# gwenzhang/GGA

Hardware: AMD Instinct MI355X
Metric: kitti_frames_per_sec_gga_train_step (higher is better)
Workload: dtype f32 tensors; products on 2 x f16 operand planes (block-scaled), f32 accumulate - measured no less accurate than fp32 kernels: per convolution 0.7 x (dense) / 0.7-1.2 x (sparse) the RMS error of an fp32 FMA chain vs float64, whole-step losses over 8 seeds <= 2.5e-5 from float64 (fp32 CPU step: <= 1.6

## Files before the change

gga_amd/_lib.py:

```python
import ctypes as C
import os
import subprocess

_HERE = os.path.dirname(os.path.abspath(__file__))
LIB_PATH = os.path.join(_HERE, 'libgga_hip.so')
ABI_VERSION = 36

_lib = None

vp, i32, i64, f32, sz = C.c_void_p, C.c_int, C.c_int64, C.c_float, C.c_size_t
I3 = C.POINTER(C.c_int32 * 3)


class VoxelParams(C.Structure):
    _fields_ = [('voxel_size', C.c_float * 3), ('pc_range', C.c_float * 6),
                ('max_points', C.c_int32), ('max_voxels', C.c_int32)]


class PfnParams(C.Structure):
    _fields_ = [('voxel_size', C.c_float * 3), ('offsets', C.c_float * 3), ('eps', C.c_float),
                ('momentum', C.c_float), ('training', C.c_int32), ('in_features', C.c_int32),
                ('channels', C.c_int32)]


# ... 52 lines not shown
CENTER_MAX_K = 512


class CenterParams(C.Structure):
    _fields_ = [('pc_range', C.c_float * 2), ('voxel_size', C.c_float * 2), ('out_size_factor', C.c_float),
                ('gaussian_overlap', C.c_float), ('min_radius', C.c_int32), ('K', C.c_int32), ('H', C.c_int32), ('W', C.c_int32),
                ('n_tasks', C.c_int32), ('n_classes', C.c_int32), ('task_classes', C.c_int32 * MAX_TASKS),
                ('task_class_base', C.c_int32 * MAX_TASKS), ('class_task', C.c_int32 * CENTER_MAX_CLASSES),
                ('class_index', C.c_int32 * CENTER_MAX_CLASSES)]


class CenterLossTask(C.Structure):
    _fields_ = [('pred', vp), ('anno_box', vp), ('mask', vp), ('loss', vp), ('grad_loss', vp), ('grad_pred', vp)]


class CenterLossTable(C.Structure):
    _fields_ = [('n_tasks', C.c_int32), ('task', CenterLossTask * MAX_TASKS)]


class CenterLossWeights(C.Structure):
    _fields_ = [('code_weights', C.c_float * 8), ('loss_weight', C.c_float)]


FPS_REGISTER_MAX_N = 20480
GROUP_MAX_SAMPLES = 256
ANCHOR_MAX_GROUPS = 16
ANCHOR_LOSS_WORKSPACE_BYTES = 24576


class AnchorParams(C.Structure):
    _fields_ = [('n_groups', C.c_int32), ('n_rot', C.c_int32), ('num_classes', C.c_int32), ('assign_per_class', C.c_int32),
                ('pos_iou_thr', C.c_float * ANCHOR_MAX_GROUPS), ('neg_iou_thr', C.c_float * ANCHOR_MAX_GROUPS),
                ('min_pos_iou', C.c_float * ANCHOR_MAX_GROUPS), ('pos_weight', C.c_float), ('dir_offset', C.c_float),
                ('dir_limit_offset', C.c_float)]


class AnchorLossParams(C.Structure):
    _fields_ = [('B', C.c_int32), ('HW', C.c_int32), ('n_anchors', C.c_int32), ('num_classes', C.c_int32),
                ('diff_rad_by_sin', C.c_int32), ('reserved', C.c_int32), ('cls_stride', C.c_int64 * 3),
                ('reg_stride', C.c_int64 * 3), ('dir_stride', C.c_int64 * 3), ('gamma', C.c_float), ('alpha', C.c_float),
                ('beta', C.c_float), ('code_weight', C.c_float * 7), ('loss_weight', C.c_float * 3)]


class LossParams(C.Structure):
    _fields_ = [('B', C.c_int32), ('K', C.c_int32), ('fm_w', C.c_int32),
                ('voxel_size', C.c_float * 2), ('out_size_factor', C.c_float),
                ('pc_range', C.c_float * 2), ('code_weights', C.c_float * 5),
                ('l1_loss_weight', C.c_float), ('w_bpl', C.c_float), ('w_srl', C.c_float),
                ('w_pal', C.c_float)]


SIGNATURES = {
    'gga_last_error': (C.c_char_p, []),
    'gga_abi_version': (i32, []),
    'gga_timing_begin': (i32, [i32, i32, i64]),
    'gga_timing_collect': (i32, [i32, vp, i32]),
    'gga_voxel_grid_size': (None, [C.POINTER(VoxelParams), C.POINTER(C.c_int32 * 3)]),
    'gga_hard_voxelize_workspace_bytes': (sz, [i32, i64]),
    'gga_hard_voxelize_batch': (i32, [vp, i32, C.POINTER(C.c_int64), i32, C.POINTER(VoxelParams),
                                       vp, vp, vp, vp, vp, sz, vp]),
    'gga_hard_voxelize_prepared': (i32, [vp, i32, C.POINTER(C.c_int64), vp, i32, C.POINTER(VoxelParams),
                                          vp, vp, vp, vp, vp, sz, vp]),
    'gga_dynamic_voxelize': (i32, [vp, i32, C.POINTER(C.c_int64), vp, i32, C.POINTER(VoxelParams), vp, vp, vp]),
    'gga_dynamic_voxel_map_workspace_bytes': (sz, [i64]),
    'gga_dynamic_voxel_map': (i32, [vp, vp, i32, i64, i32, i32, i32, i32, vp, vp, vp, vp, vp, vp, sz, vp]),
    'gga_dynamic_scatter_chunk': (i32, []),
    'gga_dynamic_scatter_workspace_bytes': (sz, [i64, i32]),
    'gga_dynamic_scatter_fwd': (i32, [vp, i32, i64, vp, vp, vp, vp, i64, i32, vp, vp, vp, sz, vp]),
    'gga_dynamic_scatter_bwd': (i32, [vp, i32, i64, vp, vp, vp, i64, i32, vp, vp]),
    'gga_dynamic_pfn_workspace_bytes': (sz, [i64]),
    'gga_dynamic_pfn_fwd': (i32, [vp, vp, i64, vp, vp, vp, vp, i64, C.POINTER(PfnParams)] + [vp] * 10 + [sz, vp]),
    'gga_dynamic_pfn_bwd': (i32, [vp, vp, i64, vp, i64, C.POINTER(PfnParams)] + [vp] * 11 + [sz, vp]),
    'gga_points_prepare_workspace_bytes': (sz, [i32, i64, i64]),
    'gga_points_prepare_batch': (i32, [vp, C.POINTER(C.c_int64), vp, C.POINTER(C.c_int64), vp, C.POINTER(C.c_int64),
                                        i32, i32, C.c_double, vp, C.POINTER(C.c_uint64), vp, vp, vp, sz, vp]),
    'gga_voxel_mean': (i32, [vp, vp, i64, i32, i32, i32, vp, vp]),
    'gga_pfn_workspace_bytes': (sz, [i64]),
    'gga_pfn_fwd': (i32, [vp, vp, vp, i64, vp, i32, C.POINTER(PfnParams), vp, vp, vp, vp, vp, vp, vp, vp, vp, sz, vp]),
    'gga_pfn_bwd': (i32, [vp, vp, vp, i64, vp, i32, C.POINTER(PfnParams), vp, vp, vp, vp, vp, vp, vp, vp, vp, vp, sz, vp]),
    'gga_pillar_scatter_map_bytes': (sz, [i32, i32, i32]),
    'gga_pillar_scatter_fwd': (i32, [vp, vp, i64, vp, i32, i32, i32, i32, i32, i32, vp, vp, vp]),
    'gga_pillar_scatter_bwd': (i32, [vp, vp, i64, vp, i32, i32, i32, i32, i32, vp, vp]),
    'gga_pillar_conv_map': (i32, [vp, i64, vp, i32, i32, i32, i32, i32, i32, i32, i32, i32, vp, vp]),
    'gga_sparse_index_bytes': (sz, [i64]),
    'gga_sparse_build_index': (i32, [vp, i64, i32, i32, i32, i32, vp, sz, vp]),
    'gga_sparse_out_index_bytes': (sz, [i64, i32]),
    'gga_sparse_out_sites_workspace_bytes': (sz, [i64, i32]),
    'gga_sparse_conv_out_sites': (i32, [vp, i64, i32, I3, I3, I3, I3, I3, vp, i64, vp, vp, sz, vp, sz, vp]),
    'gga_sparse_rulebook': (i32, [vp, i64, vp, i64, i32, I3, I3, I3, I3, I3, vp, i64, vp, i64, vp, vp, vp]),
    'gga_sparse_rowmask': (i32, [vp, i64, i32, vp, vp]),
    'gga_sparse_mask_order_workspace_bytes': (sz, [i64]),
    'gga_sparse_morton_order_workspace_bytes': (sz, [i64]),
    'gga_sparse_morton_order': (i32, [vp, i64, i32, i32, vp, vp, sz, vp]),
    'gga_sparse_mask_order': (i32, [vp, i64, i32, vp, vp, sz, vp]),
    'gga_sparse_split_weight_bytes': (sz, [i32, i32, i32]),
    'gga_sparse_conv_wgrad_workspace_bytes': (sz, [i64, i32, i32, i32]),
    'gga_dense_wgrad3x3_workspace_bytes': (sz, [i32, i32, i32, i32, i32]),
    'gga_sparse_pack_weight_planes': (i32, [vp, i32, i32, i32, i32, i32, vp, vp, vp]),
    'gga_sparse_conv_apply_tiles': (i64, [i64]),
    'gga_sparse_conv_apply_bn_bwd': (i32, [vp, vp, vp, vp, vp, i64, i32, i32, i32, i32, vp, i64, i32, vp, vp, vp, vp, i64, vp, vp, vp, vp, vp]),
    'gga_sparse_bev_nhwc_fwd': (i32, [vp, vp, i64, i32, i32, i32, i32, i32, vp, vp]),
    'gga_sparse_bev_nhwc_bwd': (i32, [vp, vp, i64, i32, i32, i32, i32, i32, vp, vp]),
    'gga_sparse_halo_tile_rows': (i64, []),
    'gga_sparse_halo_build': (i32, [vp, vp, i64, i64, i32, i32, vp, vp, vp, vp]),
    'gga_sparse_conv_apply_halo': (i32, [vp, vp, vp, vp, i32, vp, vp, i64, i64, i32, i32, i32, i32, vp, i64, i32, vp, vp, vp, vp, i64, vp, vp, vp, vp, vp]),
    'gga_sparse_conv_wgrad_planes': (i32, [vp, i64, vp, i64, vp, i64, i32, i32, i32, vp, i32, vp, vp, vp, sz, vp]),
    'gga_deconv_stream_tiles': (i64, [i64, i32, i32]),
    'gga_deconv_stream_fwd': (i32, [vp, vp, vp, vp, i32, i32, i32, i32, i32, i32, vp, vp, vp]),
    'gga_deconv_stream_bwd': (i32, [vp, vp, vp, vp, i32, i32, i32, i32, i32, i32, vp, vp]),
    'gga_absmax_bits': (i32, [vp, i64, i32, i64, vp, vp]),
    'gga_dense_conv3x3_pack_planes': (i32, [vp, i64, i64, i64, i64, i32, i32, i32, i32, vp, vp, vp]),
    'gga_dense_conv3x3_levels': (i32, [i32, vp, vp, vp, vp, i32, i32, i32, vp, i64, i32, vp, vp, vp, i32, i32, vp, vp]),
    'gga_dense_conv3x3_bn_bwd_pays': (i32, [i32, i32, i32, i32]),
    'gga_dense_conv3x3_bn_bwd_pays_planes': (i32, [i32, i32, i32, i32, i32]),
    'gga_dense_conv3x3_bn_bwd': (i32, [vp, vp, i32, i32, i32, i32, i32, vp, i64, i32, vp, i32, vp, vp, vp, i64, vp, vp, vp, vp, vp]),
    'gga_absmax_table_blocks': (i64, [i64]),
    'gga_absmax_table': (i32, [vp, i32, i64, vp, i32, vp]),
    'gga_pack_weights_table': (i32, [vp, i32, i64, i32, vp]),
    'gga_dense_wgrad3x3_block_amax': (i32, [vp, vp, i32, i32, i32, i32, i32, vp, i64, i64, i64, i64, i32, i32, vp, i32, vp, i32, vp, sz, vp]),
    'gga_dense_conv3x3_tile_rows': (i32, [i32, i32, i32, i32, i32]),
    'gga_dense_conv3x3_stat_rows': (i64, [i32, i32, i32, i32, i32, i32]),
    'gga_bn_relu_workspace_bytes': (sz, [i64, i32]),
    'gga_bn_relu_mask_bytes': (sz, [i64, i32]),
    'gga_bn_relu_fwd': (i32, [vp, vp, vp, vp, vp, vp, i64, i32, f32, f32, i32, i32, vp, i64, vp, vp, vp, i32, vp, vp, sz, vp]),
    'gga_bn_relu_bwd': (i32, [vp, i64, vp, vp, vp, vp, i64, i32, i32, i32, vp, vp, vp, vp, vp, vp, sz, vp]),
    'gga_column_sums': (i32, [vp, i64, i32, vp, vp, sz, vp]),
    'gga_bn_relu_bwd_partials': (i32, [vp, i64, vp, vp, vp, i64, i32, i32, vp, i32, vp, vp, vp, vp, vp, sz, vp]),
    'gga_gn_relu_workspace_bytes': (sz, [i32, i32]),
    'gga_gn_relu_fwd': (i32, [vp, vp, vp, i32, i64, i32, i32, f32, i32, vp, vp, vp, vp, vp, sz, vp]),
    'gga_gn_relu_bwd': (i32, [vp, vp, vp, vp, vp, i32, i64, i32, i32, i32, vp, vp, vp, vp, vp, sz, vp]),
    'gga_bn_stats': (i32, [vp, vp, vp, vp, vp, i64, i32, f32, f32, i32, vp, vp, vp, i32, i32, i32, vp, sz, vp]),
    'gga_head_conv3x3_fwd': (i32, [vp, i64, vp, vp, vp, i32, i32, i32, i32, i32, vp, vp]),
    'gga_head_conv3x3_fwd_tiles': (i32, [vp, i64, vp, vp, vp, i32, i32, i32, i32, i32, vp, vp, vp]),
    'gga_head_cell_tiles_count': (i64, [i32, i32, i32]),
    'gga_head_cell_tiles': (i32, [vp, i32, i32, i32, i32, vp, vp]),
    'gga_head_conv3x3_workspace_bytes': (sz, [i32]),
    'gga_head_conv3x3_wgrad': (i32, [vp, i64, vp, vp, i32, i32, i32, i32, i32, vp, vp, vp, sz, vp]),
    'gga_head_tail_bwd': (i32, [vp, vp, i64, vp, vp, vp, vp, i32, i32, i32, i32, i32, vp, i64, vp, vp, vp, vp, sz, vp]),
    'gga_head_tile_activity': (i32, [vp, i32, i32, i32, i32, vp, vp]),
    'gga_head_branch_bwd_workspace_bytes': (sz, [i32, i32, i32, i32]),
    'gga_head_branch_bwd': (i32, [vp, vp, i64, vp, vp, vp, vp, i32, i32, i32, i32, i32, vp, vp, vp, i64, vp, vp, vp, i32, vp, sz, vp]),
    'gga_heatmap_splat': (i32, [vp, i32, i32, i32, vp, i32, vp, vp, i32, vp]),
    'gga_focal_loss_workspace_bytes': (sz, [i64, i32]),
    'gga_focal_loss_fwd': (i32, [C.POINTER(TaskTable), f32, f32, f32, vp, sz, vp]),
    'gga_focal_loss_bwd': (i32, [C.POINTER(TaskTable), f32, f32, f32, vp]),
    'gga_gather_pred_fwd': (i32, [C.POINTER(TaskTable), i32, i32, i32, i32, vp]),
    'gga_gather_pred_bwd': (i32, [C.POINTER(TaskTable), i32, i32, i32, i32, vp]),
    'gga_box_losses_workspace_bytes': (sz, [i32, i32, i32]),
    'gga_box_losses_fwd': (i32, [C.POINTER(TaskTable), C.POINTER(LossParams), vp, sz, vp]),
    'gga_box_losses_bwd': (i32, [C.POINTER(TaskTable), i32, i32, vp]),
    'gga_center_targets': (i32, [vp, vp, vp, i32, C.POINTER(CenterParams), vp, vp, vp, vp, vp, vp, i32, vp]),
    'gga_center_reg_loss_fwd': (i32, [C.POINTER(CenterLossTable), i32, i32, C.POINTER(CenterLossWeights), vp]),
    'gga_center_reg_loss_bwd': (i32, [C.POINTER(CenterLossTable), i32, i32, C.POINTER(CenterLossWeights), vp]),
    'gga_anchor_targets_workspace_bytes': (sz, [i64, i32]),
    'gga_anchor_targets': (i32, [vp, i32, C.POINTER(AnchorParams), vp, vp, i32, vp, vp, i32, vp, vp, vp, vp, vp, vp, vp, vp, sz, vp]),
    'gga_anchor_loss_fwd': (i32, [C.POINTER(AnchorLossParams), vp, vp, vp, vp, vp, vp, vp, vp, vp, vp, vp, vp, sz, vp]),
    'gga_anchor_loss_bwd': (i32, [C.POINTER(AnchorLossParams), vp, vp, vp, vp, vp, vp, vp, vp, vp, vp, vp, vp, vp, vp, vp]),
    'gga_anchor_decode': (i32, [vp, i32, i32, vp, i32, i32, i32, vp, vp, C.POINTER(C.c_int64 * 3), vp, C.POINTER(C.c_int64 * 3), vp, vp, vp, vp]),
    'gga_box_iou_rotated': (i32, [vp, i32, vp, i32, i32, i32, vp, vp]),
    'gga_nms_rotated_workspace_bytes': (sz, [i32]),
    'gga_nms_rotated_sorted': (i32, [vp, i32, f32, i32, vp, vp, vp, sz, vp]),
    'gga_circle_nms_sorted': (i32, [vp, i32, C.c_double, i32, vp, vp, vp, sz, vp]),
    'gga_region_grow_workspace_bytes': (sz, [i64, i32]),
    'gga_region_grow': (i32, [vp, i64, i32, vp, vp, vp, i32, C.c_double, i32, vp, vp, sz, vp]),
    'gga_points_in_convex_polyhedra': (i32, [vp, i64, i32, vp, vp, i32, i32, vp, vp]),
    'gga_plane_inliers': (i32, [vp, i64, i32, vp, i32, C.c_double, vp, vp, vp]),
# ... 87 lines not shown
```

gga_amd/csrc/scatter.hip:

```cpp
#include "gga_common.h"

__global__ __launch_bounds__(256) void scatter_map_kernel(const int32_t* __restrict__ coors, int64_t m,
                                                         const int32_t* __restrict__ num_valid, int batch,
                                                         int ny, int nx, int32_t* __restrict__ cell_map) {
    const int64_t v = (int64_t)blockIdx.x * 256 + threadIdx.x;
    const int64_t lim = num_valid ? (int64_t)*num_valid : m;
    if (v >= m || v >= lim) return;
    const int4 c = reinterpret_cast<const int4*>(coors)[v];
    if ((unsigned)c.x >= (unsigned)batch || (unsigned)c.z >= (unsigned)ny || (unsigned)c.w >= (unsigned)nx) return;
    atomicMax(&cell_map[((int64_t)c.x * ny + c.z) * nx + c.w], (int32_t)v);
}

template <int UNROLL>
__global__ __launch_bounds__(256) void scatter_canvas_nchw_v1_kernel(const float* __restrict__ feats,
                                                                    int32_t* __restrict__ cell_map, int channels,
                                                                    int64_t cells, int64_t cells4_total,
                                                                    float* __restrict__ canvas) {
    const int64_t q = (int64_t)blockIdx.x * 256 + threadIdx.x;
    if (q >= cells4_total) return;
    const int64_t cells4 = cells >> 2;
    const int64_t b = q / cells4;
    const int64_t cq = q - b * cells4;
    int4* mp = reinterpret_cast<int4*>(cell_map) + q;
    const int4 idx = *mp;
// ... 286 lines not shown
    const int ky = k / kw, kx = k - ky * kw;
    int32_t v = -1;
    if (!num_valid || r < *num_valid) {
        const int4 c = coors[r];
        const int ty = c.z + ph - ky, tx = c.w + pw - kx;
        if (ty >= 0 && tx >= 0 && ty % sh == 0 && tx % sw == 0) {
            const int oy = ty / sh, ox = tx / sw;
            if (oy < oh && ox < ow) v = (c.x * oh + oy) * ow + ox;
        }
    }
    map[(int64_t)k * m + r] = v;
}

__global__ __launch_bounds__(256) void sparse_bev_nhwc_fwd_kernel(const float4* __restrict__ f, const int4* __restrict__ coors,
                                                                int64_t n, int c4n, int D, int H, int W, float* __restrict__ out) {
    const int64_t i = (int64_t)blockIdx.x * 256 + threadIdx.x;
    if (i >= n * c4n) return;
    const int64_t row = i / c4n;
    const int c4 = (int)(i - row * c4n);
    const int4 c = coors[row];
    const float4 v = f[i];
    float* dst = out + (((int64_t)c.x * H + c.z) * W + c.w) * (4 * c4n * D) + (int64_t)(4 * c4) * D + c.y;
    dst[0] = v.x; dst[D] = v.y; dst[2 * D] = v.z; dst[3 * D] = v.w;
}

__global__ __launch_bounds__(256) void sparse_bev_nhwc_bwd_kernel(const float* __restrict__ g, const int4* __restrict__ coors,
                                                                int64_t n, int c4n, int D, int H, int W, float4* __restrict__ gf) {
    const int64_t i = (int64_t)blockIdx.x * 256 + threadIdx.x;
    if (i >= n * c4n) return;
    const int64_t row = i / c4n;
    const int c4 = (int)(i - row * c4n);
    const int4 c = coors[row];
    const float* src = g + (((int64_t)c.x * H + c.z) * W + c.w) * (4 * c4n * D) + (int64_t)(4 * c4) * D + c.y;
    gf[i] = make_float4(src[0], src[D], src[2 * D], src[3 * D]);
}

extern "C" int gga_sparse_bev_nhwc_fwd(const float* feats, const int32_t* coors, int64_t n, int batch, int channels, int depth,
                                       int height, int width, float* out, void* stream_) {
    hipStream_t stream = (hipStream_t)stream_;
    GGA_REQUIRE(out && batch >= 1 && channels >= 4 && channels % 4 == 0 && depth >= 1 && height >= 1 && width >= 1 && n >= 0,
                "gga_sparse_bev_nhwc_fwd: bad sizes (channels %% 4 == 0)");
    GGA_CHECK_HIP(hipMemsetAsync(out, 0, (size_t)batch * height * width * channels * depth * sizeof(float), stream),
                  "gga_sparse_bev_nhwc_fwd: memset");
    if (n == 0) return GGA_OK;
    GGA_REQUIRE(feats && coors && ((uintptr_t)feats & 15) == 0 && ((uintptr_t)coors & 15) == 0, "gga_sparse_bev_nhwc_fwd: null or unaligned pointer");
    const int64_t total = n * (channels / 4);
    hipLaunchKernelGGL(sparse_bev_nhwc_fwd_kernel, dim3((unsigned)((total + 255) / 256)), dim3(256), 0, stream,
                       (const float4*)feats, (const int4*)coors, n, channels / 4, depth, height, width, out);
    GGA_CHECK_LAUNCH("sparse_bev_nhwc_fwd_kernel");
    return GGA_OK;
}

extern "C" int gga_sparse_bev_nhwc_bwd(const float* grad_out, const int32_t* coors, int64_t n, int batch, int channels, int depth,
                                       int height, int width, float* grad_feats, void* stream_) {
    hipStream_t stream = (hipStream_t)stream_;
    GGA_REQUIRE(batch >= 1 && channels >= 4 && channels % 4 == 0 && depth >= 1 && height >= 1 && width >= 1 && n >= 0,
                "gga_sparse_bev_nhwc_bwd: bad sizes (channels %% 4 == 0)");
    if (n == 0) return GGA_OK;
    GGA_REQUIRE(grad_out && coors && grad_feats && ((uintptr_t)grad_feats & 15) == 0 && ((uintptr_t)coors & 15) == 0,
                "gga_sparse_bev_nhwc_bwd: null or unaligned pointer");
    const int64_t total = n * (channels / 4);
    hipLaunchKernelGGL(sparse_bev_nhwc_bwd_kernel, dim3((unsigned)((total + 255) / 256)), dim3(256), 0, stream, grad_out,
                       (const int4*)coors, n, channels / 4, depth, height, width, (float4*)grad_feats);
    GGA_CHECK_LAUNCH("sparse_bev_nhwc_bwd_kernel");
    return GGA_OK;
}

extern "C" int gga_pillar_conv_map(const int32_t* coors, int64_t m, const int32_t* num_valid, int batch, int ny, int nx,
                                   int kh, int kw, int stride_h, int stride_w, int pad_h, int pad_w, int32_t* map,
                                   void* stream) {
    GGA_REQUIRE(coors && map, "gga_pillar_conv_map: null pointer argument");
    GGA_REQUIRE(m >= 0 && batch >= 1 && ny >= 1 && nx >= 1 && kh >= 1 && kw >= 1 && kh * kw <= 65535 && stride_h >= 1 &&
                    stride_w >= 1 && pad_h >= 0 && pad_w >= 0,
                "gga_pillar_conv_map: bad sizes");
    const int oh = (ny + 2 * pad_h - kh) / stride_h + 1, ow = (nx + 2 * pad_w - kw) / stride_w + 1;
    GGA_REQUIRE(oh >= 1 && ow >= 1 && (int64_t)batch * oh * ow < 2147483647ll, "gga_pillar_conv_map: output %dx%d", oh, ow);
    if (m == 0) return GGA_OK;
    hipLaunchKernelGGL(pillar_conv_map_kernel, dim3((unsigned)((m + 255) / 256), kh * kw), dim3(256), 0,
                       (hipStream_t)stream, (const int4*)coors, m, num_valid, kh, kw, stride_h, stride_w, pad_h, pad_w,
                       oh, ow, map);
    GGA_CHECK_LAUNCH("pillar_conv_map_kernel");
    return GGA_OK;
}
```

gga_amd/pillar_conv.py:

```python
import torch
from torch import nn

from . import _lib
from . import functional as F
from . import gather_gemm as G
from ._lib import check


class PillarSupport:
    __slots__ = ('feats', 'coors', 'num_valid')

    def __init__(self, feats, coors, num_valid):
        self.feats, self.coors, self.num_valid = feats, coors, num_valid


def eligible(conv, canvas):
    sup = getattr(canvas, 'pillar_support', None)
    return (sup is not None and type(conv) is nn.Conv2d and conv.bias is None and conv.groups == 1
            and tuple(conv.dilation) == (1, 1) and conv.padding_mode == 'zeros' and not isinstance(conv.padding, str)
            and canvas.is_cuda and canvas.dtype == torch.float32 and torch.is_grad_enabled()
            and (sup.feats.requires_grad or conv.weight.requires_grad)
            and conv.in_channels <= 128 and conv.out_channels <= 128 and conv.in_channels % 4 == 0
            and canvas.is_contiguous(memory_format=torch.channels_last))


class _PillarConv2d(torch.autograd.Function):
    @staticmethod
    def forward(ctx, feats, weight, canvas, coors, num_valid, stride, padding):
        from . import strided_conv
        kh, kw = weight.shape[2:]
        if (strided_conv.ENABLED and kh == kw and stride[0] == stride[1] and padding[0] == padding[1] and stride[0] > 1
                and kh <= 5 and weight.shape[0] % 4 == 0):
            B, Ci, ny, nx = canvas.shape
            bk = strided_conv.book(B, ny, nx, kh, stride[0], padding[0], canvas.device)
            y, stats = G.apply(canvas.permute(0, 2, 3, 1).reshape(-1, Ci), bk.fwd, weight.detach().permute(2, 3, 1, 0).reshape(kh * kw, Ci, -1),
                               bk.n_out, planes=G.planes(), x_amax=G.amax(feats.detach().contiguous()), want_stats=True)
            y = y.view(B, bk.Ho, bk.Wo, -1).permute(0, 3, 1, 2)
        else:
            y = torch.conv2d(canvas, weight, None, stride, padding)
            stats = torch.empty(0, dtype=torch.float64, device=y.device)
        ctx.save_for_backward(feats, weight, coors, num_valid)
        ctx.geom = (tuple(canvas.shape), stride, padding)
        ctx.mark_non_differentiable(stats)
        ctx.set_materialize_grads(False)
        return y, stats

    @staticmethod
    def backward(ctx, gy, _gstats=None):
        feats, w, coors, num_valid = ctx.saved_tensors
        (B, Ci, ny, nx), (sh, sw), (ph, pw) = ctx.geom
        Co, _, kh, kw = w.shape
        kvol, m = kh * kw, feats.shape[0]
        gy = gy.contiguous(memory_format=torch.channels_last)
        rows = gy.permute(0, 2, 3, 1).reshape(-1, Co)
        feats = feats.contiguous()
        L = _lib.lib()
        nbr = torch.empty((kvol, m), dtype=torch.int32, device=gy.device)
        check(L.gga_pillar_conv_map(F._p(coors), m, F._p(num_valid), B, ny, nx, kh, kw, sh, sw, ph, pw, F._p(nbr),
                                    F._stream()), 'gga_pillar_conv_map')
        gx = gw = None
        if ctx.needs_input_grad[0]:
            rb = G.Rulebook(nbr)
            wk = w.permute(2, 3, 0, 1).reshape(kvol, Co, Ci).contiguous()
            gx = G.apply(rows, rb, wk, m, planes=3)
        if ctx.needs_input_grad[1]:
            gw = G.wgrad(rows, feats, nbr, m, planes=3).view(kh, kw, Co, Ci).permute(2, 3, 0, 1)
        return gx, gw, None, None, None, None, None


def pillar_conv2d(canvas, conv):
    sup = canvas.pillar_support
    coors = sup.coors if sup.coors.dtype == torch.int32 else sup.coors.int()
    y, stats = _PillarConv2d.apply(sup.feats, conv.weight, canvas.detach(), coors.contiguous(), sup.num_valid,
                                   tuple(conv.stride), tuple(conv.padding))
    if stats.numel():
        F.attach_bn_partials(y, stats)
    return y
```

gga_amd/strided_conv.py:

```python
import ctypes as C
import os

import torch
from torch import nn

from . import _lib
from . import functional as F
from . import gather_gemm as G
from ._lib import check

ENABLED = True
STREAM = os.environ.get('GGA_DECONV_STREAM', '1') != '0'
STREAM_OFF = set()
_BOOKS = {}


class _Book:

    def __init__(self, B, H, W, k, s, p, device):
        Ho, Wo = (H + 2 * p - k) // s + 1, (W + 2 * p - k) // s + 1
        self.Ho, self.Wo, self.kvol = Ho, Wo, k * k
        self.n_in, self.n_out = B * H * W, B * Ho * Wo
        self._geom = (B, H, W, k, s, p, device)

# ... 106 lines not shown
    from . import dense_conv, weight_bank
    L = _lib.lib()
    B, cout, Hs, Ws = gy.shape
    H, W = Hs // s, Ws // s
    cin = weight.shape[0]
    w_koi = weight.detach().permute(2, 3, 1, 0)
    if dense_conv.RANGE_GUARD.armed:
        dense_conv.RANGE_GUARD.record(w_koi)
    ops = [weight_bank.gather_operand(w_koi, 2, c0, min(c0 + 128, cin)) for c0 in range(0, cin, 128)]
    g_amax = G.amax(gy) if g_amax is None else g_amax
    gx = torch.empty((B, H, W, cin), dtype=torch.float32, device=gy.device)
    check(L.gga_deconv_stream_bwd(F._p(_rows(gy)), _block_pointers([op for op, _ in ops]), F._p(g_amax), F._p(ops[0][1]), B, H, W,
                                  cin, cout, s, F._p(gx), F._stream()), 'gga_deconv_stream_bwd')
    return gx


class _Deconv(torch.autograd.Function):

    @staticmethod
    def forward(ctx, x, weight, s):
        B, cin, H, W = x.shape
        w = weight.detach()
        x_amax = G.amax(x)
        if _stream_form(cin, weight.shape[1], s, False):
            y, stats = _stream_fwd(x, weight, s, x_amax)
            ctx.save_for_backward(x, weight)
            ctx.s, ctx.amax = s, (x_amax, None)
            ctx.mark_non_differentiable(stats)
            ctx.set_materialize_grads(False)
            return y.permute(0, 3, 1, 2), stats
        bk = book(B, H * s, W * s, s, s, 0, x.device)
        y, stats = G.apply(_rows(x), bk.bwd, w.permute(2, 3, 0, 1), bk.n_in, planes=G.planes(), x_amax=x_amax, want_stats=True, bank=True)
        ctx.save_for_backward(x, weight)
        ctx.s, ctx.amax = s, (x_amax, None)
        ctx.mark_non_differentiable(stats)
        ctx.set_materialize_grads(False)
        return y.view(B, H * s, W * s, -1).permute(0, 3, 1, 2), stats

    @staticmethod
    def backward(ctx, gy, _gstats=None):
        x, weight = ctx.saved_tensors
        s = ctx.s
        B, cin, H, W = x.shape
        cout = weight.shape[1]
        gy = gy.contiguous(memory_format=torch.channels_last)
        g_rows = _rows(gy)
        gx = gw = None
        x_amax, w_amax = ctx.amax if G.planes() == 2 else (None, None)
        g_amax = G.amax(gy)
        stream = _stream_form(cin, cout, s, True)
        if not stream or ctx.needs_input_grad[1]:
            bk = book(B, H * s, W * s, s, s, 0, x.device)
        if ctx.needs_input_grad[0]:
            if stream:
                gx = _stream_bwd(gy, weight, s, g_amax).permute(0, 3, 1, 2)
            else:
                w = weight.detach()
                gx = G.apply(g_rows, bk.fwd, w.permute(2, 3, 1, 0), bk.n_out, planes=G.planes(), x_amax=g_amax, bank=True)
                gx = gx.view(B, H, W, cin).permute(0, 3, 1, 2)
        if ctx.needs_input_grad[1]:
            gw = G.wgrad(g_rows, _rows(x), bk.fwd.nbr, bk.n_out, planes=G.planes(), x_amax=g_amax, g_amax=x_amax).view(s, s, cout, cin).permute(3, 2, 0, 1)
        return gx, gw, None


def _common(m, x):
    return (ENABLED and max(m.in_channels, m.out_channels) <= 256 and m.bias is None and m.groups == 1 and m.dilation == (1, 1) and x.is_cuda and x.dtype == torch.float32
            and x.dim() == 4 and x.is_contiguous(memory_format=torch.channels_last) and m.in_channels % 4 == 0
            and m.out_channels % 4 == 0 and x.shape[0] * x.shape[2] * x.shape[3] * max(m.stride) ** 2 < 2 ** 31)


def eligible(m, x):
    if type(m) is nn.Conv2d:
        k, s, p = m.kernel_size, m.stride, m.padding
        return (_common(m, x) and m.padding_mode == 'zeros' and k[0] == k[1] and s[0] == s[1] and p[0] == p[1] and k[0] <= 5
                and (s[0] > 1 or k[0] == 1) and isinstance(p[0], int))
    if type(m) is nn.ConvTranspose2d:
        k, s = m.kernel_size, m.stride
        return (_common(m, x) and k == s and k[0] == k[1] and k[0] <= 5 and m.padding == (0, 0) and m.output_padding == (0, 0))
    return False


def conv(x, m):
    if type(m) is nn.Conv2d:
        y, stats = _StridedConv.apply(x, m.weight, m.kernel_size[0], m.stride[0], m.padding[0])
    else:
        y, stats = _Deconv.apply(x, m.weight, m.stride[0])
    F.attach_bn_partials(y, stats)
    return y
```

include/gga_hip.h:

```cpp
#ifndef GGA_HIP_H_
#define GGA_HIP_H_

#include <stddef.h>
#include <stdint.h>

#ifdef __cplusplus
extern "C" {
#endif

typedef enum {
    GGA_OK = 0,
    GGA_ERR_INVALID_ARG = -1,
    GGA_ERR_WORKSPACE = -2,
    GGA_ERR_LAUNCH = -3
} gga_status;

const char* gga_last_error(void);
int gga_abi_version(void);

enum {
    GGA_TIME_SCATTER_FWD = 0,
    GGA_TIME_DENSE_CONV = 1,
    GGA_TIME_SPARSE_CONV = 2,
    GGA_TIME_SPARSE_WGRAD = 3,
// ... 27 lines not shown
                               void* workspace, size_t workspace_bytes, void* stream);

size_t gga_points_prepare_workspace_bytes(int n_frames, int64_t total_rows, int64_t max_frame_rows);
int gga_points_prepare_batch(const float* scene, const int64_t* scene_offsets_host, const float* sampled,
                             const int64_t* sampled_offsets_host, const double* centers_xy,
                             const int64_t* center_offsets_host, int n_frames, int ndim, double min_distance,
                             const float* pc_range_dev, const uint64_t* shuffle_seeds_host, float* out_points,
                             int32_t* out_counts, void* workspace, size_t workspace_bytes, void* stream);

int gga_voxel_mean(const float* voxels, const int32_t* num_points, int64_t m, int max_points,
                   int ndim, int num_features, float* out, void* stream);

int gga_dynamic_voxelize(const float* points, int ndim, const int64_t* offsets_host, const int32_t* counts_dev, int batch,
                         const gga_voxel_params* prm, int32_t* coors, uint32_t* keys, void* stream);

size_t gga_dynamic_voxel_map_workspace_bytes(int64_t n_points);
int gga_dynamic_voxel_map(const uint32_t* keys, const int32_t* coors, int coor_cols, int64_t n_points, int batch, int grid_x,
                          int grid_y, int grid_z, int32_t* voxel_coors, int32_t* voxel_start, int32_t* order,
                          int32_t* point2voxel, int32_t* counts, void* workspace, size_t workspace_bytes, void* stream);

enum { GGA_DYNAMIC_MEAN = 0, GGA_DYNAMIC_MAX = 1 };
int gga_dynamic_scatter_chunk(void);
size_t gga_dynamic_scatter_workspace_bytes(int64_t n_points, int channels);
int gga_dynamic_scatter_fwd(const float* feats, int channels, int64_t n_points, const int32_t* order,
                            const int32_t* point2voxel, const int32_t* voxel_start, const int32_t* counts, int64_t out_rows,
                            int mode, float* out, int32_t* argmax, void* workspace, size_t workspace_bytes, void* stream);
int gga_dynamic_scatter_bwd(const float* grad_out, int channels, int64_t n_points, const int32_t* point2voxel,
                            const int32_t* voxel_start, const int32_t* argmax, int64_t out_rows, int mode, float* grad_in,
                            void* stream);

typedef struct {
    float voxel_size[3];
    float offsets[3];
    float eps, momentum;
    int32_t training;
    int32_t in_features;
    int32_t channels;
} gga_pfn_params;

size_t gga_pfn_workspace_bytes(int64_t m);
int gga_pfn_fwd(const float* voxels, const int32_t* num_points, const int32_t* coors, int64_t m,
                const int32_t* num_valid, int max_points, const gga_pfn_params* prm, const float* weight, const float* gamma,
                const float* beta, float* running_mean, float* running_var, float* out,
                uint8_t* argmax, double* saved, void* workspace, size_t workspace_bytes,
                void* stream);
int gga_pfn_bwd(const float* voxels, const int32_t* num_points, const int32_t* coors, int64_t m,
                const int32_t* num_valid, int max_points, const gga_pfn_params* prm, const float* weight, const float* gamma,
                const float* out, const uint8_t* argmax, const double* saved, const float* grad_out,
                float* grad_weight, float* grad_gamma, float* grad_beta, void* workspace,
                size_t workspace_bytes, void* stream);

size_t gga_dynamic_pfn_workspace_bytes(int64_t n_points);
int gga_dynamic_pfn_fwd(const float* points, const int32_t* coors, int64_t n_points, const int32_t* order,
                        const int32_t* point2voxel, const int32_t* voxel_start, const int32_t* counts, int64_t out_rows,
                        const gga_pfn_params* prm, const float* weight, const float* gamma, const float* beta,
                        float* running_mean, float* running_var, float* out, int32_t* argmax, float* mean, double* saved,
                        void* workspace, size_t workspace_bytes, void* stream);
int gga_dynamic_pfn_bwd(const float* points, const int32_t* coors, int64_t n_points, const int32_t* counts, int64_t out_rows,
                        const gga_pfn_params* prm, const float* weight, const float* gamma, const float* out,
                        const int32_t* argmax, const float* mean, const double* saved, const float* grad_out,
                        float* grad_weight, float* grad_gamma, float* grad_beta, void* workspace, size_t workspace_bytes,
                        void* stream);

enum { GGA_LAYOUT_NCHW = 0, GGA_LAYOUT_NHWC = 1 };

size_t gga_pillar_scatter_map_bytes(int batch, int ny, int nx);

int gga_pillar_scatter_fwd(const float* feats, const int32_t* coors, int64_t m,
                           const int32_t* num_valid, int batch, int channels, int ny, int nx,
                           int layout, int unique_coors, int32_t* cell_map, float* canvas, void* stream);

int gga_pillar_scatter_bwd(const float* grad_canvas, const int32_t* coors, int64_t m,
                           const int32_t* num_valid, int batch, int channels, int ny, int nx,
                           int layout, float* grad_feats, void* stream);

int gga_sparse_bev_nhwc_fwd(const float* feats, const int32_t* coors, int64_t n, int batch, int channels, int depth, int height,
                            int width, float* out, void* stream);
int gga_sparse_bev_nhwc_bwd(const float* grad_out, const int32_t* coors, int64_t n, int batch, int channels, int depth,
                            int height, int width, float* grad_feats, void* stream);

int gga_pillar_conv_map(const int32_t* coors, int64_t m, const int32_t* num_valid, int batch, int ny, int nx,
                        int kh, int kw, int stride_h, int stride_w, int pad_h, int pad_w, int32_t* map,
                        void* stream);


size_t gga_sparse_index_bytes(int64_t n);
int gga_sparse_build_index(const int32_t* coors, int64_t n, int B, int D, int H, int W, void* index,
                           size_t index_bytes, void* stream);

size_t gga_sparse_out_index_bytes(int64_t n_in, int kvol);
size_t gga_sparse_out_sites_workspace_bytes(int64_t n_in, int kvol);
int gga_sparse_conv_out_sites(const int32_t* in_coors, int64_t n_in, int B, const int32_t in_dhw[3],
                              const int32_t kernel[3], const int32_t stride[3], const int32_t pad[3],
                              int32_t out_dhw[3], int32_t* out_coors, int64_t cap_out, int32_t* n_out,
                              void* out_index, size_t out_index_bytes, void* workspace,
                              size_t workspace_bytes, void* stream);

int gga_sparse_rulebook(const int32_t* out_coors, int64_t n_out, const int32_t* in_coors, int64_t n_in,
                        int B, const int32_t in_dhw[3], const int32_t out_dhw[3], const int32_t kernel[3],
                        const int32_t stride[3], const int32_t pad[3], const void* in_index,
                        int64_t in_index_n, const void* out_index, int64_t out_index_n, int32_t* nbr,
                        int32_t* nbr_t, void* stream);

int gga_sparse_rowmask(const int32_t* map, int64_t n_rows, int kvol, uint32_t* mask, void* stream);
size_t gga_sparse_morton_order_workspace_bytes(int64_t n_rows);
int gga_sparse_morton_order(const int32_t* coors, int64_t n_rows, int batch_size, int max_extent, int32_t* order,
                            void* workspace, size_t workspace_bytes, void* stream);
size_t gga_sparse_mask_order_workspace_bytes(int64_t n_rows);
int gga_sparse_mask_order(const uint32_t* mask, int64_t n_rows, int kvol, int32_t* order, void* workspace,
                          size_t workspace_bytes, void* stream);

size_t gga_sparse_split_weight_bytes(int kvol, int cin, int cout);

int64_t gga_dense_conv3x3_stat_rows(int B, int H, int W, int cout, int planes, int n_slices);
int gga_dense_conv3x3_tile_rows(int B, int H, int W, int cout, int planes);

int gga_absmax_bits(const float* x, int64_t rows, int width, int64_t row_stride, uint32_t* out_bits, void* stream);
typedef struct {
    const float* src;
    uint16_t* dst;
    const uint32_t* amax;
    int64_t s_k0, s_k1, s_c, s_col;
    int64_t first;
    int32_t kw, kvol, n_c, n_col, c0, col0, n_in, co, layout, reverse;
} GgaPackEntry;
typedef struct {
    const float* src;
    uint32_t* slot;
    int64_t n;
    int64_t first_block;
} GgaAmaxEntry;
int64_t gga_absmax_table_blocks(int64_t n);
int gga_absmax_table(const GgaAmaxEntry* table_device, int n_entries, int64_t n_blocks, uint32_t* slots, int n_slots, void* stream);
int gga_pack_weights_table(const GgaPackEntry* table_device, int n_entries, int64_t total, int planes, void* stream);
int gga_sparse_pack_weight_planes(const float* weight, int kvol, int cin, int cout, int transpose, int planes,
                                  const uint32_t* amax_weight, void* packed, void* stream);
int64_t gga_sparse_conv_apply_tiles(int64_t n_rows);
int gga_sparse_conv_apply_bn_bwd(const float* x, const int32_t* map, const void* split_weight, const int32_t* perm,
                                 const uint32_t* rowmask, int64_t n_rows, int kvol, int cin, int cout, int flip, float* y,
                                 int64_t y_row_stride, int planes, const uint32_t* amax_x, const uint32_t* amax_weight,
                                 double* stats, const float* bn_x, int64_t bn_x_row_stride, const float* bn_gamma,
                                 const float* bn_beta, const float* bn_mean, const float* bn_invstd, void* stream);
int64_t gga_sparse_halo_tile_rows(void);
int gga_sparse_halo_build(const int32_t* nbr, const int32_t* tile_rows, int64_t n_rows, int64_t n_tiles, int kvol,
                          int halo_capacity, int32_t* halo_rows, int32_t* halo_counts, uint16_t* local_map, void* stream);
int gga_sparse_conv_apply_halo(const float* x, const void* split_weight, const int32_t* tile_rows,
                               const int32_t* halo_counts, int halo_capacity, const int32_t* halo_rows,
                               const uint16_t* local_map, int64_t n_rows, int64_t n_tiles, int kvol, int cin, int cout, int flip,
                               float* y, int64_t y_row_stride, int planes, const uint32_t* amax_x, const uint32_t* amax_weight,
                               double* stats, const float* bn_x, int64_t bn_x_row_stride, const float* bn_gamma,
                               const float* bn_beta, const float* bn_mean, const float* bn_invstd, void* stream);
size_t gga_sparse_conv_wgrad_workspace_bytes(int64_t n_rows, int kvol, int cin, int cout);
int gga_sparse_conv_wgrad_planes(const float* x, int64_t x_row_stride, const float* grad_out, int64_t grad_out_row_stride,
                                 const int32_t* nbr, int64_t n_rows, int kvol, int cin, int cout, float* grad_weight,
                                 int planes, const uint32_t* amax_x, const uint32_t* amax_grad_out, void* workspace,
                                 size_t workspace_bytes, void* stream);
int64_t gga_deconv_stream_tiles(int64_t n_pixels, int cin, int s);
int gga_deconv_stream_fwd(const float* x, const void* const* weight_blocks, const uint32_t* amax_x,
                          const uint32_t* amax_weight, int B, int h, int w, int cin, int cout, int s, float* y, double* stats,
                          void* stream);
int gga_deconv_stream_bwd(const float* gy, const void* const* weight_blocks, const uint32_t* amax_gy,
                          const uint32_t* amax_weight, int B, int h, int w, int cin, int cout, int s, float* gx, void* stream);
int gga_dense_conv3x3_pack_planes(const float* weight, int64_t stride_co, int64_t stride_ci, int64_t stride_ky,
                                  int64_t stride_kx, int cin, int cout, int backward, int planes,
                                  const uint32_t* amax_weight, void* packed, void* stream);
int gga_dense_conv3x3_bn_bwd_pays_planes(int B, int H, int W, int cout, int planes);
// ... 402 lines not shown
```

tools_dev/deconv_stream_calls.py:

```python
import collections
import csv
import glob
import os
import re
import sys

FLOOR = 5.5e12
B, H, W = 16, 248, 216
N1, N2, N3 = B * H * W, B * H * W // 4, B * H * W // 16
LAYERS = {'D1': (N1, 64, N1, 128), 'D2': (N2, 128, N1, 128), 'D3': (N3, 256, N1, 128),
          'opener1': (4 * N1, 64, N1, 64), 'opener2': (N1, 64, N2, 128), 'opener3': (N2, 128, N3, 256)}


def last_step(d):
    f = max(glob.glob(os.path.join(d, '**', '*kernel_trace.csv'), recursive=True), key=os.path.getmtime)
    rows = list(csv.DictReader(open(f)))
    rows.sort(key=lambda r: int(r['Start_Timestamp']))
    opt = [i for i, r in enumerate(rows) if 'multi_tensor_apply' in r['Kernel_Name']]
    ends = [opt[i] for i in range(len(opt)) if i + 1 == len(opt) or opt[i + 1] - opt[i] > 50]
    return rows[ends[-3] + 1:ends[-1] + 1]


def us(r):
    return (int(r['End_Timestamp']) - int(r['Start_Timestamp'])) / 1e3


def short(name):
    return re.sub(r'^void ', '', name.split('(')[0])[:52]


def label(calls):
    out, seen = [], collections.Counter()
    fwd_order = ['opener1', 'opener2', 'opener3', 'opener3', 'D1', 'D2', 'D3']
    wgrad_order = ['D3', 'D3', 'D2', 'D1', 'opener3', 'opener3', 'opener2']
    n_fwd = 0
    for r in calls:
        name, wg = r['Kernel_Name'], int(r['Workgroup_Size_X'])
        tiles = int(r['Grid_Size_X']) // wg
        m = re.search(r'deconv_stream_(fwd|bwd)_kernel<([0-9, ]+)>', name)
        if 'NP = 3' in name or re.search(r', 3>', name):
            out.append(('pillars', 'weight gradient' if 'wgrad' in name else 'backward-data'))
        elif m and m.group(1) == 'fwd':
            out.append(({6696: 'D1', 1674: 'D2', 837: 'D3'}.get(tiles, '?'), 'forward'))
        elif m:
            out.append(({'1, 1, 64': 'D1', '1, 2, 128': 'D2', '2, 2, 128': 'D3'}.get(m.group(2), '?'), 'backward-data'))
        elif 'wgrad' in name:
            out.append((wgrad_order[seen['w']] if seen['w'] < len(wgrad_order) else '?', 'weight gradient'))
            seen['w'] += 1
        elif seen['w'] == 0 and n_fwd < len(fwd_order):
            out.append((fwd_order[n_fwd], 'forward'))
            n_fwd += 1
        else:
            have = {l for l, d in out if d == 'backward-data'}
            neck, opener = {419: ('D3', 'D3'), 1674: ('D2', 'opener3'), 6696: ('D1', 'opener2')}.get(tiles, ('?', '?'))
            out.append((neck if neck not in have or tiles == 419 else opener, 'backward-data'))
    return out


def need_bytes(layer, direction, half=False):
    if layer not in LAYERS or direction == 'weight gradient':
        return None
    n_in, cin, n_out, cout = LAYERS[layer]
    d = 2 if half else 1
    return 4 * (n_in * cin // d + n_out * cout) if direction == 'backward-data' else 4 * (n_in * cin + n_out * cout // d)


def main():
    step = last_step(sys.argv[1])
    pat = re.compile(r'sp_conv_x9_kernel|sp_conv_wgrad_x9_kernel|deconv_stream_')
    calls = [r for r in step if pat.search(r['Kernel_Name'])]
    print(f'{"us":>8}  {"tiles":>6}  {"layer":8} {"direction":15} {"need MB":>8} {"TB/s":>6} {"of floor":>8}  kernel')
    for r, (layer, direction) in zip(calls, label(calls)):
        t = us(r)
        half = 'sp_conv_x9' in r['Kernel_Name'] and ((layer == 'D3' and direction == 'backward-data') or (layer == 'opener3' and direction == 'forward'))
        nb = need_bytes(layer, direction, half)
        rate = f'{nb / t / 1e6:6.2f} {nb / FLOOR / (t * 1e-6):8.2f}' if nb else f'{"":6} {"":8}'
        mb = f'{nb / 1e6:8.0f}' if nb else f'{"":8}'
        print(f'{t:8.1f}  {int(r["Grid_Size_X"]) // int(r["Workgroup_Size_X"]):6d}  {layer:8} {direction:15} {mb} {rate}  {short(r["Kernel_Name"])}')
    tot = collections.defaultdict(float)
    for r in step:
        tot[short(r['Kernel_Name'])] += us(r)
    other = collections.defaultdict(float)
    two = len(sys.argv) > 2
    if two:
        for r in last_step(sys.argv[2]):
            other[short(r['Kernel_Name'])] += us(r)
    print(f'\nstep: {sum(tot.values()) / 1e3:.3f} ms busy in {len(step)} launches' + (f'; other trace {sum(other.values()) / 1e3:.3f} ms' if two else ''))
    for k in sorted(set(tot) | set(other), key=lambda k: -max(tot[k], other[k])):
        if max(tot[k], other[k]) >= 20 or abs(tot[k] - other[k]) >= 30:
            print(f'{tot[k] / 1e3:9.3f} ms' + (f' {other[k] / 1e3:9.3f} ms {(tot[k] - other[k]) / 1e3:+8.3f}' if two else '') + f'  {k}')


if __name__ == '__main__':
    main()
```

Measured before the change: 553.3.

## Gather first strided conv directly from pillar rows via remapped rulebook

Adds a pillar forward-book: a dense cell-to-pillar table is built and used to remap the strided conv's neighbor rulebook from canvas cells to pillar row indices, with a per-row tap mask. The first strided conv then gathers from the compact pillar feature rows instead of the dense NHWC canvas, so it no longer reads mostly-empty canvas memory. The price is three extra small kernels (table fill, set, remap) plus a table workspace the size of the canvas grid. It is on by default and also covers the no-grad path.

```diff
diff --git a/gga_amd/_lib.py b/gga_amd/_lib.py
--- a/gga_amd/_lib.py
+++ b/gga_amd/_lib.py
@@ -158,6 +158,8 @@
     'gga_pillar_scatter_fwd': (i32, [vp, vp, i64, vp, i32, i32, i32, i32, i32, i32, vp, vp, vp]),
     'gga_pillar_scatter_bwd': (i32, [vp, vp, i64, vp, i32, i32, i32, i32, i32, vp, vp]),
     'gga_pillar_conv_map': (i32, [vp, i64, vp, i32, i32, i32, i32, i32, i32, i32, i32, i32, vp, vp]),
+    'gga_pillar_fwd_book_workspace_bytes': (sz, [i32, i32, i32]),
+    'gga_pillar_fwd_book': (i32, [vp, i64, vp, i32, i32, i32, vp, i64, i32, vp, vp, vp, sz, vp]),
     'gga_sparse_index_bytes': (sz, [i64]),
     'gga_sparse_build_index': (i32, [vp, i64, i32, i32, i32, i32, vp, sz, vp]),
     'gga_sparse_out_index_bytes': (sz, [i64, i32]),
diff --git a/gga_amd/csrc/scatter.hip b/gga_amd/csrc/scatter.hip
--- a/gga_amd/csrc/scatter.hip
+++ b/gga_amd/csrc/scatter.hip
@@ -392,3 +392,77 @@
     GGA_CHECK_LAUNCH("pillar_conv_map_kernel");
     return GGA_OK;
 }
+
+__global__ __launch_bounds__(256) void pillar_table_fill_kernel(int4* __restrict__ table4, int64_t total4) {
+    const int64_t t = (int64_t)blockIdx.x * 256 + threadIdx.x;
+    if (t < total4) table4[t] = make_int4(-1, -1, -1, -1);
+}
+
+__global__ __launch_bounds__(256) void pillar_table_set_kernel(const int4* __restrict__ coors, int64_t m,
+                                                              const int32_t* __restrict__ num_valid, int batch, int ny,
+                                                              int nx, int32_t* __restrict__ table) {
+    const int64_t v = (int64_t)blockIdx.x * 256 + threadIdx.x;
+    const int64_t lim = num_valid ? (int64_t)*num_valid : m;
+    if (v >= m || v >= lim) return;
+    const int4 c = coors[v];
+    if ((unsigned)c.x >= (unsigned)batch || (unsigned)c.z >= (unsigned)ny || (unsigned)c.w >= (unsigned)nx) return;
+    table[((int64_t)c.x * ny + c.z) * nx + c.w] = (int32_t)v;
+}
+
+#define PB_TAPS 9
+__global__ __launch_bounds__(256) void pillar_fwd_book_kernel(const int32_t* __restrict__ nbr, int64_t n_out, int kvol,
+                                                             const int32_t* __restrict__ table, int64_t cells,
+                                                             int32_t* __restrict__ nbr_p, uint32_t* __restrict__ mask_p) {
+    const int64_t row = (int64_t)blockIdx.x * 256 + threadIdx.x;
+    if (row >= n_out) return;
+    uint32_t mask = 0;
+    for (int k0 = 0; k0 < kvol; k0 += PB_TAPS) {
+        int32_t cell[PB_TAPS], p[PB_TAPS];
+#pragma unroll
+        for (int j = 0; j < PB_TAPS; ++j) cell[j] = k0 + j < kvol ? nbr[(int64_t)(k0 + j) * n_out + row] : -1;
+#pragma unroll
+        for (int j = 0; j < PB_TAPS; ++j) p[j] = (cell[j] >= 0 && cell[j] < cells) ? table[cell[j]] : -1;
+#pragma unroll
+        for (int j = 0; j < PB_TAPS; ++j)
+            if (k0 + j < kvol) {
+                nbr_p[(int64_t)(k0 + j) * n_out + row] = p[j];
+                mask |= (p[j] >= 0 ? 1u : 0u) << (k0 + j);
+            }
+    }
+    mask_p[row] = mask;
+}
+
+extern "C" size_t gga_pillar_fwd_book_workspace_bytes(int batch, int ny, int nx) {
+    if (batch < 1 || ny < 1 || nx < 1) return 0;
+    return gga_align_up((size_t)batch * ny * nx * sizeof(int32_t), 256);
+}
+
+extern "C" int gga_pillar_fwd_book(const int32_t* coors, int64_t m, const int32_t* num_valid, int batch, int ny, int nx,
+                                   const int32_t* nbr, int64_t n_out, int kvol, int32_t* nbr_p, uint32_t* mask_p,
+                                   void* workspace, size_t workspace_bytes, void* stream_) {
+    hipStream_t stream = (hipStream_t)stream_;
+    GGA_REQUIRE(nbr && nbr_p && mask_p && workspace && (m == 0 || coors), "gga_pillar_fwd_book: null pointer argument");
+    GGA_REQUIRE(m >= 0 && batch >= 1 && ny >= 1 && nx >= 1 && n_out >= 1 && kvol >= 1 && kvol <= 32 &&
+                    (int64_t)batch * ny * nx < 2147483647ll && n_out < 2147483647ll && m < 2147483647ll,
+                "gga_pillar_fwd_book: bad sizes (m=%lld batch=%d ny=%d nx=%d n_out=%lld kvol=%d; kvol <= 32)", (long long)m,
+                batch, ny, nx, (long long)n_out, kvol);
+    GGA_REQUIRE(((uintptr_t)workspace & 15) == 0 && ((uintptr_t)coors & 15) == 0,
+                "gga_pillar_fwd_book: workspace and coors must be 16-byte aligned");
+    const size_t need = gga_pillar_fwd_book_workspace_bytes(batch, ny, nx);
+    GGA_REQUIRE(workspace_bytes >= need, "gga_pillar_fwd_book: workspace too small (%zu < %zu bytes)", workspace_bytes, need);
+    const int64_t cells = (int64_t)batch * ny * nx;
+    int32_t* table = (int32_t*)workspace;
+    const int64_t total4 = (int64_t)(need / 16);
+    hipLaunchKernelGGL(pillar_table_fill_kernel, dim3((unsigned)((total4 + 255) / 256)), dim3(256), 0, stream, (int4*)table,
+                       total4);
+    GGA_CHECK_LAUNCH("pillar_table_fill_kernel");
+    if (m > 0) {
+        hipLaunchKernelGGL(pillar_table_set_kernel, dim3((unsigned)((m + 255) / 256)), dim3(256), 0, stream,
+                           (const int4*)coors, m, num_valid, batch, ny, nx, table);
+        GGA_CHECK_LAUNCH("pillar_table_set_kernel");
+    }
+    hipLaunchKernelGGL(pillar_fwd_book_kernel, dim3((unsigned)((n_out + 255) / 256)), dim3(256), 0, stream, nbr, n_out, kvol,
+                       (const int32_t*)table, cells, nbr_p, mask_p);
+    GGA_CHECK_LAUNCH("pillar_fwd_book_kernel");
+    return GGA_OK;
+}
diff --git a/gga_amd/pillar_conv.py b/gga_amd/pillar_conv.py
--- a/gga_amd/pillar_conv.py
+++ b/gga_amd/pillar_conv.py
@@ -1,3 +1,5 @@
+import os
+
 import torch
 from torch import nn
 
@@ -5,6 +7,41 @@
 from . import functional as F
 from . import gather_gemm as G
 from ._lib import check
+
+
+FWD_BOOK = os.environ.get('GGA_PILLAR_FWD_BOOK', '1') != '0'
+
+
+class _FwdBook:
+    __slots__ = ('nbr', 'mask', 'perm', 'coors')
+
+    def __init__(self, nbr, mask, perm):
+        self.nbr, self.mask, self.perm, self.coors = nbr, mask, perm, None
+
+
+def fwd_book(bk, coors, num_valid, B, ny, nx):
+    L = _lib.lib()
+    kvol, n_out = bk.fwd.nbr.shape
+    nbr_p = torch.empty((kvol, n_out), dtype=torch.int32, device=coors.device)
+    mask_p = torch.empty(n_out, dtype=torch.int32, device=coors.device)
+    nbytes = int(L.gga_pillar_fwd_book_workspace_bytes(B, ny, nx))
+    table = F._workspace('pillar_fwd_book', nbytes, coors.device)
+    check(L.gga_pillar_fwd_book(F._p(coors), coors.shape[0], F._p(num_valid), B, ny, nx, F._p(bk.fwd.nbr), n_out, kvol, F._p(nbr_p),
+                                F._p(mask_p), F._p(table), nbytes, F._stream()), 'gga_pillar_fwd_book')
+    return _FwdBook(nbr_p, mask_p, bk.fwd.perm)
+
+
+def fwd_book_form(sup, cin, kvol):
+    return (FWD_BOOK and sup is not None and kvol <= 32 and sup.feats.dim() == 2 and sup.feats.shape[0] >= 1 and sup.feats.shape[1] == cin
+            and sup.feats.dtype == torch.float32 and sup.coors.shape[0] == sup.feats.shape[0])
+
+
+def conv_no_grad(x, m, bk):
+    sup = x.pillar_support
+    coors = (sup.coors if sup.coors.dtype == torch.int32 else sup.coors.int()).contiguous()
+    B, _, ny, nx = x.shape
+    return G.apply(sup.feats.detach().contiguous(), fwd_book(bk, coors, sup.num_valid, B, ny, nx), m.weight.detach().permute(2, 3, 1, 0),
+                   bk.n_out, planes=G.planes(), x_amax=G.amax(x), want_stats=True, bank=True)
 
 
 class PillarSupport:
@@ -33,8 +70,13 @@
                 and kh <= 5 and weight.shape[0] % 4 == 0):
             B, Ci, ny, nx = canvas.shape
             bk = strided_conv.book(B, ny, nx, kh, stride[0], padding[0], canvas.device)
-            y, stats = G.apply(canvas.permute(0, 2, 3, 1).reshape(-1, Ci), bk.fwd, weight.detach().permute(2, 3, 1, 0).reshape(kh * kw, Ci, -1),
-                               bk.n_out, planes=G.planes(), x_amax=G.amax(feats.detach().contiguous()), want_stats=True)
+            rows_f = feats.detach().contiguous()
+            if fwd_book_form(PillarSupport(rows_f, coors, num_valid), Ci, kh * kw):
+                x_rows, rb = rows_f, fwd_book(bk, coors, num_valid, B, ny, nx)
+            else:
+                x_rows, rb = canvas.permute(0, 2, 3, 1).reshape(-1, Ci), bk.fwd
+            y, stats = G.apply(x_rows, rb, weight.detach().permute(2, 3, 1, 0).reshape(kh * kw, Ci, -1),
+                               bk.n_out, planes=G.planes(), x_amax=G.amax(rows_f), want_stats=True)
             y = y.view(B, bk.Ho, bk.Wo, -1).permute(0, 3, 1, 2)
         else:
             y = torch.conv2d(canvas, weight, None, stride, padding)
diff --git a/gga_amd/strided_conv.py b/gga_amd/strided_conv.py
--- a/gga_amd/strided_conv.py
+++ b/gga_amd/strided_conv.py
@@ -212,7 +212,15 @@
 
 def conv(x, m):
     if type(m) is nn.Conv2d:
-        y, stats = _StridedConv.apply(x, m.weight, m.kernel_size[0], m.stride[0], m.padding[0])
+        from . import pillar_conv
+        k, s, p = m.kernel_size[0], m.stride[0], m.padding[0]
+        if not torch.is_grad_enabled() and pillar_conv.fwd_book_form(getattr(x, 'pillar_support', None), m.in_channels, k * k):
+            B, _, H, W = x.shape
+            bk = book(B, H, W, k, s, p, x.device)
+            y, stats = pillar_conv.conv_no_grad(x, m, bk)
+            y = y.view(B, bk.Ho, bk.Wo, -1).permute(0, 3, 1, 2)
+        else:
+            y, stats = _StridedConv.apply(x, m.weight, k, s, p)
     else:
         y, stats = _Deconv.apply(x, m.weight, m.stride[0])
     F.attach_bn_partials(y, stats)
diff --git a/include/gga_hip.h b/include/gga_hip.h
--- a/include/gga_hip.h
+++ b/include/gga_hip.h
@@ -133,6 +133,11 @@
 int gga_pillar_conv_map(const int32_t* coors, int64_t m, const int32_t* num_valid, int batch, int ny, int nx,
                         int kh, int kw, int stride_h, int stride_w, int pad_h, int pad_w, int32_t* map,
                         void* stream);
+
+size_t gga_pillar_fwd_book_workspace_bytes(int batch, int ny, int nx);
+int gga_pillar_fwd_book(const int32_t* coors, int64_t m, const int32_t* num_valid, int batch, int ny, int nx,
+                        const int32_t* nbr, int64_t n_out, int kvol, int32_t* nbr_p, uint32_t* mask_p, void* workspace,
+                        size_t workspace_bytes, void* stream);
 
 
 size_t gga_sparse_index_bytes(int64_t n);
diff --git a/tools_dev/deconv_stream_calls.py b/tools_dev/deconv_stream_calls.py
--- a/tools_dev/deconv_stream_calls.py
+++ b/tools_dev/deconv_stream_calls.py
@@ -8,6 +8,7 @@
 FLOOR = 5.5e12
 B, H, W = 16, 248, 216
 N1, N2, N3 = B * H * W, B * H * W // 4, B * H * W // 16
+HELPERS = re.compile(r'pillar_table_(fill|set)_kernel|pillar_fwd_book_kernel|scatter_map_reset_kernel')
 LAYERS = {'D1': (N1, 64, N1, 128), 'D2': (N2, 128, N1, 128), 'D3': (N3, 256, N1, 128),
           'opener1': (4 * N1, 64, N1, 64), 'opener2': (N1, 64, N2, 128), 'opener3': (N2, 128, N3, 256)}
 
@@ -37,6 +38,9 @@
     for r in calls:
         name, wg = r['Kernel_Name'], int(r['Workgroup_Size_X'])
         tiles = int(r['Grid_Size_X']) // wg
+        if HELPERS.search(name):
+            out.append(('opener1', 'pillar map'))
+            continue
         m = re.search(r'deconv_stream_(fwd|bwd)_kernel<([0-9, ]+)>', name)
         if 'NP = 3' in name or re.search(r', 3>', name):
             out.append(('pillars', 'weight gradient' if 'wgrad' in name else 'backward-data'))
@@ -57,9 +61,11 @@
     return out
 
 
-def need_bytes(layer, direction, half=False):
-    if layer not in LAYERS or direction == 'weight gradient':
+def need_bytes(layer, direction, half=False, pillars=0):
+    if layer not in LAYERS or direction in ('weight gradient', 'pillar map'):
         return None
+    if layer == 'opener1' and direction == 'forward' and pillars:
+        return 4 * (pillars * 64 + 10 * N1 + N1 * 64)
     n_in, cin, n_out, cout = LAYERS[layer]
     d = 2 if half else 1
     return 4 * (n_in * cin // d + n_out * cout) if direction == 'backward-data' else 4 * (n_in * cin + n_out * cout // d)
@@ -68,12 +74,13 @@
 def main():
     step = last_step(sys.argv[1])
     pat = re.compile(r'sp_conv_x9_kernel|sp_conv_wgrad_x9_kernel|deconv_stream_')
-    calls = [r for r in step if pat.search(r['Kernel_Name'])]
+    calls = [r for r in step if pat.search(r['Kernel_Name']) or HELPERS.search(r['Kernel_Name'])]
+    pillars = max([int(r['Grid_Size_X']) for r in calls if 'pillar_table_set_kernel' in r['Kernel_Name']] or [0])
     print(f'{"us":>8}  {"tiles":>6}  {"layer":8} {"direction":15} {"need MB":>8} {"TB/s":>6} {"of floor":>8}  kernel')
     for r, (layer, direction) in zip(calls, label(calls)):
         t = us(r)
         half = 'sp_conv_x9' in r['Kernel_Name'] and ((layer == 'D3' and direction == 'backward-data') or (layer == 'opener3' and direction == 'forward'))
-        nb = need_bytes(layer, direction, half)
+        nb = need_bytes(layer, direction, half, pillars)
         rate = f'{nb / t / 1e6:6.2f} {nb / FLOOR / (t * 1e-6):8.2f}' if nb else f'{"":6} {"":8}'
         mb = f'{nb / 1e6:8.0f}' if nb else f'{"":8}'
         print(f'{t:8.1f}  {int(r["Grid_Size_X"]) // int(r["Workgroup_Size_X"]):6d}  {layer:8} {direction:15} {mb} {rate}  {short(r["Kernel_Name"])}')
```

After: 554.0, median of 4. About the same (+0.1%).
